# qianduoduolr/FGVC

Measured on AMD Instinct MI355X. Metric: frames/sec + ms/corr-volume, 480p 8-frame clip, 1/2/4/8 MI355X, higher is better.
Workload: dtype f16 + fp6 (e2m3) MFMA operands, f32 accumulate; top-k near-ties re-scored in f64 from f32 features

## Files before the change

### fgvc_amd/csrc/common.hpp

```cpp
#pragma once

#include <hip/hip_runtime.h>
#include <math.h>
#include <stdint.h>
#include <stdio.h>

#include "../../include/fgvc_hip.h"
#include "sortnet.hpp"

namespace fgvc {

typedef float f32x4 __attribute__((ext_vector_type(4)));
typedef float f32x16 __attribute__((ext_vector_type(16)));
typedef short bf16x8 __attribute__((ext_vector_type(8)));

constexpr int WAVE = 64;
constexpr int IDX_EMPTY = 0x7fffffff;

void set_error(const char* fmt, ...);

#define FGVC_REQUIRE(cond, code, ...)        \
  do {                                       \
    if (!(cond)) {                           \
      ::fgvc::set_error(__VA_ARGS__);        \
// ... 193 lines not shown
typedef int fgvc_i32x8 __attribute__((ext_vector_type(8)));
typedef int fgvc_i32x4 __attribute__((ext_vector_type(4)));

constexpr int F8_AX = 7, F8_BX = 3;
constexpr int F8_AW = 2, F8_BW = 9;

__device__ __forceinline__ void split_f16_4(const f32x4& x, float s, uint2& hw, uint32_t& l8, uint32_t& h8, uint2& lw, bool& ovf) {
  typedef _Float16 f16x4 __attribute__((ext_vector_type(4)));
  f16x4 h, l;
  float hf[4], lf[4];
#pragma unroll
  for (int i = 0; i < 4; ++i) {
    const float xs = x[i] * s;
    ovf |= fabsf(xs) > 57344.f;
    const float c = __builtin_amdgcn_fmed3f(xs, -65504.f, 65504.f);
    h[i] = (_Float16)c;
    hf[i] = (float)h[i];
    lf[i] = c - hf[i];
    l[i] = (_Float16)lf[i];
  }
  hw = __builtin_bit_cast(uint2, h);
  lw = __builtin_bit_cast(uint2, l);
  constexpr float SA = 1.0f / (float)(1 << F8_AX), SB = (float)(1 << F8_BX);
  int a = __builtin_amdgcn_cvt_pk_fp8_f32(__builtin_amdgcn_fmed3f(hf[0] * SA, -448.f, 448.f), __builtin_amdgcn_fmed3f(hf[1] * SA, -448.f, 448.f), 0, false);
  a = __builtin_amdgcn_cvt_pk_fp8_f32(__builtin_amdgcn_fmed3f(hf[2] * SA, -448.f, 448.f), __builtin_amdgcn_fmed3f(hf[3] * SA, -448.f, 448.f), a, true);
  int b = __builtin_amdgcn_cvt_pk_fp8_f32(lf[0] * SB, lf[1] * SB, 0, false);
  b = __builtin_amdgcn_cvt_pk_fp8_f32(lf[2] * SB, lf[3] * SB, b, true);
  h8 = (uint32_t)a;
  l8 = (uint32_t)b;
}

typedef int fgvc_i32x6 __attribute__((ext_vector_type(6)));
typedef int fgvc_i32x16 __attribute__((ext_vector_type(16)));
__device__ __forceinline__ void split_f16f6_chunk(const f32x4 (&v)[4], float s, int h, uint2 (&hw)[4], fgvc_i32x4& main6, fgvc_i32x4& tail6,
                                                  bool& ovf, float lo = -65504.f) {
  typedef _Float16 f16x2 __attribute__((ext_vector_type(2)));
  unsigned A[8], B[8];
  float mc = 0.f, md = 0.f;
#pragma unroll
  for (int g = 0; g < 4; ++g)
#pragma unroll
    for (int j = 0; j < 2; ++j) {
      const float c0 = __builtin_amdgcn_fmed3f(v[g][2 * j] * s, lo, 65504.f);
      const float c1 = __builtin_amdgcn_fmed3f(v[g][2 * j + 1] * s, lo, 65504.f);
      mc = fmaxf(fmaxf(mc, fabsf(c0)), fabsf(c1));
      f16x2 hp, lp;
      hp[0] = (_Float16)c0;
      hp[1] = (_Float16)c1;
      const float d0 = c0 - (float)hp[0], d1 = c1 - (float)hp[1];
      md = fmaxf(fmaxf(md, fabsf(d0)), fabsf(d1));
      lp[0] = (_Float16)(d0 * 2048.f);
      lp[1] = (_Float16)(d1 * 2048.f);
      A[2 * g + j] = __builtin_bit_cast(unsigned, hp);
      B[2 * g + j] = __builtin_bit_cast(unsigned, lp);
    }
  ovf |= mc > 57344.f;
  const float mh = (float)(_Float16)mc;
  const float ml = md * 2048.f;
#pragma unroll
  for (int g = 0; g < 4; ++g) hw[g] = {A[2 * g], A[2 * g + 1]};
#pragma unroll
  for (int r = 0; r < 8; ++r) {
    const auto t = __builtin_amdgcn_permlane32_swap(A[r], B[r], false, false);
    A[r] = t[0]; B[r] = t[1];
  }
  const auto tm = __builtin_amdgcn_permlane32_swap(__builtin_bit_cast(unsigned, mh), __builtin_bit_cast(unsigned, ml), false, false);
  const unsigned mu = tm[0] > tm[1] ? tm[0] : tm[1];
  const float m16 = (float)(_Float16)__builtin_bit_cast(float, mu);
  const unsigned mb = __builtin_bit_cast(unsigned, m16);
  int field = (int)(mb >> 23) - 2 + ((mb & 0x7fffffu) > 0x700000u ? 1 : 0);
  field = field < 32 ? 32 : field;
  fgvc_i32x16 T;
#pragma unroll
  for (int g = 0; g < 4; ++g)
#pragma unroll
    for (int j = 0; j < 2; ++j) {
      T[4 * g + j] = (int)A[2 * g + j];
      T[4 * g + 2 + j] = (int)B[2 * g + j];
    }
  fgvc_i32x6 c6;
  const unsigned sc_bits = (unsigned)field << 23;
  asm volatile("v_cvt_scalef32_pk32_fp6_f16 %0, %1, %2" : "=&v"(c6) : "v"(T), "v"(sc_bits));
  main6 = {c6[0], c6[1], c6[2], c6[3]};
  tail6 = {c6[4], c6[5], field - (h ? 11 : 0), 0};
}

__device__ __forceinline__ void lds_barrier() { asm volatile("s_waitcnt lgkmcnt(0)\n\ts_barrier" ::: "memory"); }

__host__ __device__ __forceinline__ int imin(int a, int b) { return a < b ? a : b; }
__host__ __device__ __forceinline__ int imax(int a, int b) { return a > b ? a : b; }
__host__ __device__ __forceinline__ int cdiv(int a, int b) { return (a + b - 1) / b; }

}
```

### fgvc_amd/csrc/conv_split.hip

```cpp
#include "common.hpp"

namespace fgvc {

struct ConvSplitParams {
  const uint16_t* x;
  const uint16_t* w;
  const float* bias;
  const float* residual;
  uint16_t* y_split;
  float* y_f32;
  int N, H, W, Hp, Wp, Cin, Cout, relu;
  int n_ty, n_tx;
  int debug;
  float acc_scale;
  float out_scale;
  int out_fmt;
  int* overflow;
  const uint16_t* x2;
  const uint16_t* w2;
  int Cin2;
  unsigned char* y_bank;
  int bank_normalize;
  int bank_row_bytes;
};
// ... 830 lines not shown
  for (int i = 0; i < 4; ++i) {
    ph |= n6_code(hf[i] * ih) << (6 * i);
    pl |= n6_code(lf[i] * il) << (6 * i);
  }
  const int v = lane >> 4, hi = (lane >> 1) & 1, pi = ((lane >> 2) & 3) * 2 + (lane & 1);
  const int w = pi < 6 ? pi : 0;
  const int pa = (4 * w) / 3, oa = 32 * w - 24 * pa;
  const int base = (lane & ~13) ;
  const int la = base + 4 * (pa >> 1) + (pa & 1), lb = base + 4 * ((pa + 1) >> 1) + ((pa + 1) & 1);
  const unsigned ha = __shfl(ph, la), hb = __shfl(ph, lb), qa = __shfl(pl, la), qb = __shfl(pl, lb);
  const unsigned wh = (ha >> oa) | (hb << (24 - oa)), wl = (qa >> oa) | (qb << (24 - oa));
  if (pi < 4) {
    *reinterpret_cast<unsigned*>(row + 512 + 32 * v + 16 * hi + 4 * pi) = wh;
    *reinterpret_cast<unsigned*>(row + 704 + 32 * v + 16 * hi + 4 * pi) = wl;
  } else if (pi < 6) {
    *reinterpret_cast<unsigned*>(row + 640 + 32 * (v >> 1) + 16 * hi + 8 * (v & 1) + 4 * (pi - 4)) = wh;
    *reinterpret_cast<unsigned*>(row + 832 + 32 * (v >> 1) + 16 * hi + 8 * (v & 1) + 4 * (pi - 4)) = wl;
  } else if (pi == 6) {
    row[896 + 16 * hi + v] = (unsigned char)(sh + 127 - 4);
  } else {
    row[896 + 16 * hi + 4 + v] = (unsigned char)(sl + 127 - 4);
  }
  if (lane < 2) *reinterpret_cast<unsigned long long*>(row + 904 + 16 * lane) = 0ull;
  else if (lane < 26) *reinterpret_cast<unsigned*>(row + 928 + 4 * (lane - 2)) = 0u;
}

static int g_conv_debug = 0;
void set_conv_debug(int v) { g_conv_debug = v; }
static int g_conv_narrow = 1;
void set_conv_narrow(int v) { g_conv_narrow = v; }
static int g_conv_cot_cap = 0;
void set_conv_cot_cap(int v) { g_conv_cot_cap = v; }

template <int COT, int OUT_FMT, bool RES, bool F32OUT, bool GENERIC, bool BANK = false, int CIN_TAG = 0>
__global__ __launch_bounds__(256, 1) void conv256p_kernel(ConvSplitParams p) {
  constexpr int NA = COT / 64, PPW = NA * 2;
  constexpr int TROWS = 8, PATCHB = (TROWS + 2) * CV_PW * 128, SLOTB = COT * 128, NPIECE = (TROWS + 2) * 5;
  __shared__ __attribute__((aligned(16))) unsigned char smem[PATCHB + 3 * SLOTB + COT * 4];
  unsigned char* patch = smem;
  unsigned char* wring = smem + PATCHB;
  float* bias_lds = reinterpret_cast<float*>(smem + PATCHB + 3 * SLOTB);
  const long long t_begin = __builtin_amdgcn_s_memtime();
  const int tid = threadIdx.x, lane = tid & 63;
  const int wave = __builtin_amdgcn_readfirstlane(tid >> 6);
  const int ch = wave & 1, pr = wave >> 1;
  const int n = lane & 31, h = lane >> 5;
  const int d_row = lane >> 3, d_slot = lane & 7;
  int bid = blockIdx.x;
  const int nimg = bid / (p.n_ty * p.n_tx);
  bid -= nimg * p.n_ty * p.n_tx;
  const int ty = bid / p.n_tx, tx = bid - ty * p.n_tx;
  const int y0 = ty * TROWS, x0 = tx * 32;
  const int co_base = blockIdx.y * COT;
  const int nchunk = p.Cin / 32;
  const uint32_t pixb = (uint32_t)nchunk * 128u;

  const uint32_t w_lane_off = (uint32_t)(d_row * 128 + ((d_slot ^ (d_row >> 1)) << 4));
  const uint32_t wo[2] = {w_lane_off, w_lane_off ^ 64u};
  const uint32_t ring_lds = lds_addr(wring), patch_lds = lds_addr(patch);
  const uint32_t wl = ring_lds + (uint32_t)((ch * (COT / 2) + n) * 128) + ((((uint32_t)h) ^ (uint32_t)((n >> 1) & 7)) << 4);
  uint32_t pl[3][2];
#pragma unroll
  for (int dx = 0; dx < 3; ++dx)
#pragma unroll
    for (int par = 0; par < 2; ++par) {
      const uint32_t key = (uint32_t)((((n + dx) >> 1) & 7) ^ (4 * par));
      pl[dx][par] = patch_lds + (uint32_t)((4 * pr * CV_PW + n + dx) * 128) + ((((uint32_t)h) ^ key) << 4);
    }
  const uint32_t pf_lane_off = (uint32_t)d_row * pixb + (uint32_t)((d_slot ^ (d_row >> 1)) << 4);
  const uint32_t lane16 = (uint32_t)lane * 16u;
  int ptab;
  {
    const int k = lane & 15, i = imin(wave + 4 * k, NPIECE - 1);
    const int prow = i / 5, pc0 = (i - prow * 5) * 8;
    const int goff = (int)((uint32_t)(prow * p.Wp + pc0) * pixb);
    const int ldst = (prow * CV_PW + pc0) * 128;
    const int key = ((prow + (pc0 >> 3)) & 1) << 6;
    ptab = lane < 16 ? goff : lane < 32 ? ldst : key;
  }
  const unsigned char* xb_tile = reinterpret_cast<const unsigned char*>(p.x) + (uint32_t)((nimg * p.Hp + y0) * p.Wp + x0) * pixb;
  const unsigned char* wb_tile = reinterpret_cast<const unsigned char*>(p.w) + (uint32_t)(co_base * 128);
  const uint32_t piece_off = (uint32_t)(wave * PPW * 1024);
  auto weight_base = [&](int chunk, int tap) { return wb_tile + (uint32_t)((tap * nchunk + chunk) * p.Cout * 128); };
  auto weight_piece = [&](const unsigned char* base, uint32_t dst, int j) {
    const unsigned char* src = base + piece_off + (uint32_t)(j * 1024);
    const uint32_t d = dst + piece_off + (uint32_t)(j * 1024);
    asm volatile("s_mov_b32 m0, %2\n\ts_nop 0\n\tglobal_load_lds_dwordx4 %0, %1" ::"v"(wo[j & 1]), "s"(src), "s"(d) : "memory");
  };

  if (tid < COT / 4) reinterpret_cast<f32x4*>(bias_lds)[tid] = reinterpret_cast<const f32x4*>(p.bias + co_base)[tid];
  for (int i = wave; i < NPIECE; i += 4) {
    const int prow = i / 5, pc0 = (i - prow * 5) * 8;
    const int P = prow * CV_PW + pc0 + d_row;
    const int sl = d_slot ^ ((P >> 1) & 7);
    const size_t gpix = ((size_t)nimg * p.Hp + (y0 + prow)) * p.Wp + (x0 + pc0 + d_row);
    conv_lds_dma_16(reinterpret_cast<const unsigned char*>(p.x) + gpix * pixb + sl * 16, lds_addr(patch + (prow * CV_PW + pc0) * 128));
  }
#pragma unroll
  for (int j = 0; j < PPW; ++j) weight_piece(weight_base(0, 0), ring_lds, j);
#pragma unroll
  for (int j = 0; j < PPW; ++j) weight_piece(weight_base(0, 1), ring_lds + SLOTB, j);

  __builtin_amdgcn_s_waitcnt(0x0F70);

  const long long t_loop0 = __builtin_amdgcn_s_memtime();
  {
    const size_t wb64 = (size_t)wb_tile, xb64 = (size_t)xb_tile;
    const int s_tap = __builtin_amdgcn_readfirstlane(nchunk * p.Cout * 128), s_chunk = __builtin_amdgcn_readfirstlane(p.Cout * 128);
    const int s_nchunk = __builtin_amdgcn_readfirstlane(nchunk), s_ring = __builtin_amdgcn_readfirstlane((int)ring_lds);
    const int s_patch = __builtin_amdgcn_readfirstlane((int)patch_lds), s_piece = __builtin_amdgcn_readfirstlane((int)piece_off);
    typedef int i32x2 __attribute__((ext_vector_type(2)));
    const i32x2 s_wb = {__builtin_amdgcn_readfirstlane((int)(uint32_t)wb64), __builtin_amdgcn_readfirstlane((int)(uint32_t)(wb64 >> 32))};
    const i32x2 s_xb = {__builtin_amdgcn_readfirstlane((int)(uint32_t)xb64), __builtin_amdgcn_readfirstlane((int)(uint32_t)(xb64 >> 32))};
    typedef int i32x2_t __attribute__((ext_vector_type(2)));
    i32x2_t loop_cycles;
    const int nchunk2 = p.x2 ? p.Cin2 / 32 : 0;
    const uint32_t pixb2 = (uint32_t)nchunk2 * 128u;
    const uint32_t pf_lane_off2 = (uint32_t)d_row * pixb2 + (uint32_t)((d_slot ^ (d_row >> 1)) << 4);
    int ptab2;
    {
      const int k2 = lane & 15, i2 = imin(wave + 4 * k2, NPIECE - 1);
      const int prow = i2 / 5, pc0 = (i2 - prow * 5) * 8;
      const int goff = (int)((uint32_t)(prow * p.Wp + pc0) * pixb2);
// ... 5 lines not shown
    const int s_last2 = __builtin_amdgcn_readfirstlane(nchunk2 ? nchunk - 1 : -1), s_nchunk2 = __builtin_amdgcn_readfirstlane(nchunk2);
#define C256P_INPUTS                                                                                                              \
  "{v232}"(wl), "{v233}"(pl[0][0]), "{v234}"(pl[0][1]), "{v235}"(pl[1][0]), "{v236}"(pl[1][1]), "{v237}"(pl[2][0]), "{v238}"(pl[2][1]),     \
      "{v239}"(wo[0]), "{v240}"(wo[1]), "{v241}"(pf_lane_off), "{v242}"(lane16), "{v243}"(ptab), "{v244}"(pf_lane_off2), "{v245}"(ptab2),  \
      "{s[20:21]}"(s_wb), "{s22}"(s_tap), "{s23}"(s_chunk), "{s[24:25]}"(s_xb), "{s26}"(s_nchunk), "{s27}"(s_ring), "{s28}"(s_patch),      \
      "{s29}"(s_piece), "{s46}"(s_last2), "{s[48:49]}"(s_w2b), "{s[50:51]}"(s_x2b), "{s52}"(s_nchunk2)
    if constexpr (COT == 256) {
#include "conv256p_loop.inc"
    } else {
#include "conv128p_loop.inc"
    }
#undef C256P_INPUTS
    if ((p.debug & 8) && blockIdx.x == 300 && blockIdx.y == 0 && lane == 0 && p.y_split) {
      long long* o = reinterpret_cast<long long*>(p.y_split) + wave * 8;
      o[4] = (long long)(uint32_t)loop_cycles.x | ((long long)loop_cycles.y << 32);
      o[5] = nchunk * 9 + nchunk2;
      o[0] = t_loop0 - t_begin;
    }
  }
  f32x16 acc[NA][4];
  if constexpr (NA == 4)
    asm volatile(""
                 : "={a[0:15]}"(acc[0][0]), "={a[16:31]}"(acc[0][1]), "={a[32:47]}"(acc[0][2]), "={a[48:63]}"(acc[0][3]), "={a[64:79]}"(acc[1][0]),
                   "={a[80:95]}"(acc[1][1]), "={a[96:111]}"(acc[1][2]), "={a[112:127]}"(acc[1][3]), "={a[128:143]}"(acc[NA - 2][0]),
                   "={a[144:159]}"(acc[NA - 2][1]), "={a[160:175]}"(acc[NA - 2][2]), "={a[176:191]}"(acc[NA - 2][3]), "={a[192:207]}"(acc[NA - 1][0]),
                   "={a[208:223]}"(acc[NA - 1][1]), "={a[224:239]}"(acc[NA - 1][2]), "={a[240:255]}"(acc[NA - 1][3]));
  else
    asm volatile(""
                 : "={a[0:15]}"(acc[0][0]), "={a[16:31]}"(acc[0][1]), "={a[32:47]}"(acc[0][2]), "={a[48:63]}"(acc[0][3]), "={a[64:79]}"(acc[1][0]),
                   "={a[80:95]}"(acc[1][1]), "={a[96:111]}"(acc[1][2]), "={a[112:127]}"(acc[1][3]));

  int lane_e;
  asm volatile("v_mbcnt_lo_u32_b32 %0, -1, 0\n\tv_mbcnt_hi_u32_b32 %0, -1, %0" : "=v"(lane_e));
  {
  int lane = lane_e, n = lane & 31, h = lane >> 5;
  int Wp_e = __builtin_amdgcn_readfirstlane(p.Wp);
  asm volatile("" : "+s"(Wp_e));
  constexpr int RPW = 4, CW = COT / 2, RB = CW * 4, RS = RB + 16, LPR = RB / 16, RPI = 64 / LPR;
  static_assert(4 * 32 * RS <= PATCHB + 3 * SLOTB, "epilogue staging");
  __syncthreads();
  long long ts0 = __builtin_amdgcn_s_memtime(), ts1 = 0, ts2 = 0, ts3 = 0, ts4 = 0;
  unsigned char* tile = smem + wave * (32 * RS);
  const int co_w = co_base + ch * CW;
  int mv_row = lane / LPR, mv_col = (lane % LPR) * 16;
  auto row_fence = [&]() { asm volatile("" : "+v"(n), "+v"(h), "+v"(mv_row), "+v"(mv_col)); };
  auto wave_sync = [&]() { asm volatile("s_waitcnt lgkmcnt(0)" ::: "memory"); };
  constexpr int RSLOTS = RB / 16, RPIECES = 32 * RB / 1024, RPPP = 1024 / RB;
  static_assert(4 * 32 * RS + 4 * 32 * RB <= PATCHB + 3 * SLOTB, "residual tiles");
  unsigned char* rtile = smem + 4 * (32 * RS) + wave * (32 * RB);
  const bool has_res = GENERIC || BANK ? p.residual != nullptr : RES;
  auto residual_dma = [&](int b_) {
    const int y_ = y0 + RPW * pr + b_;
    if (!has_res || b_ >= RPW || y_ >= p.H) return;
    const unsigned char* src = reinterpret_cast<const unsigned char*>(p.residual + (((size_t)nimg * p.H + y_) * p.W + x0) * p.Cout + co_w);
    const int pmax = p.W - 1 - x0;
#pragma unroll
    for (int j = 0; j < RPIECES; ++j) {
      const int pp = j * RPPP + (lane * 16) / RB, ps = ((lane * 16) % RB) / 16;
      const uint32_t voff = (uint32_t)(imin(pp, pmax) * p.Cout * 4 + ((ps ^ (pp & (RSLOTS - 1))) << 4));
      conv_lds_dma_16s(voff, src, lds_addr(rtile + j * 1024));
    }
  };
  auto residual_wait = [&](int stores_behind) {
    if (x0 + 32 > p.W || stores_behind == 0) asm volatile("s_waitcnt vmcnt(0)" ::: "memory");
    else if (stores_behind == 32 / RPI) asm volatile("s_waitcnt vmcnt(%0)" ::"n"(32 / RPI) : "memory");
    else asm volatile("s_waitcnt vmcnt(%0)" ::"n"(2 * (32 / RPI)) : "memory");
  };
  auto residual_at = [&](int cw) {
    return *reinterpret_cast<const f32x4*>(rtile + n * RB + ((((cw * 4) >> 4) ^ (n & (RSLOTS - 1))) << 4));
  };
  residual_dma(0);
  const bool tile_full = x0 + 32 <= p.W;
  auto store_rows = [&](unsigned char* dst) {
    unsigned char* d0 = dst + (size_t)mv_row * p.Cout * 4 + mv_col;
    const unsigned char* t0 = tile + mv_row * RS + mv_col;
    if (tile_full) {
#pragma unroll
      for (int i = 0; i < 32 / RPI; ++i) *reinterpret_cast<uint4*>(d0 + (size_t)(i * RPI) * p.Cout * 4) = *reinterpret_cast<const uint4*>(t0 + i * RPI * RS);
    } else {
#pragma unroll
      for (int i = 0; i < 32 / RPI; ++i)
        if (x0 + i * RPI + mv_row < p.W) *reinterpret_cast<uint4*>(d0 + (size_t)(i * RPI) * p.Cout * 4) = *reinterpret_cast<const uint4*>(t0 + i * RPI * RS);
    }
  };
  if constexpr (BANK) {
    {
      constexpr int BK_RS = 1024 + 16;
      static_assert(COT == 256 && 2 * 32 * BK_RS <= PATCHB + 3 * SLOTB, "bank staging");
      unsigned char* rows = smem + pr * (32 * BK_RS);
      float* part = reinterpret_cast<float*>(rows);
      long long bts[6] = {}, bt_begin = 0;
#pragma unroll
      for (int b = 0; b < RPW; ++b) {
        row_fence();
        const int y = y0 + RPW * pr + b;
        const bool row_ok = y < p.H;
        if (b == 1) bt_begin = __builtin_amdgcn_s_memtime();
        if (b == 2) bts[4] = __builtin_amdgcn_s_memtime();
        const size_t fpix0 = ((size_t)nimg * p.H + imin(y, p.H - 1)) * p.W + x0;
        if (has_res && row_ok) residual_wait(b == 0 || 32 / RPI != 16 ? 0 : (p.bank_row_bytes > 1024 ? 32 : 16));
        f32x4 v[NA][4];
#pragma unroll
        for (int a = 0; a < NA; ++a)
#pragma unroll
          for (int g = 0; g < 4; ++g) {
            const int cw = a * 32 + 8 * g + 4 * h;
            const f32x4 bv = *reinterpret_cast<const f32x4*>(bias_lds + ch * CW + cw);
            v[a][g] = {fmaf(acc[a][b][4 * g + 0], p.acc_scale, bv.x), fmaf(acc[a][b][4 * g + 1], p.acc_scale, bv.y),
                         fmaf(acc[a][b][4 * g + 2], p.acc_scale, bv.z), fmaf(acc[a][b][4 * g + 3], p.acc_scale, bv.w)};
            if (has_res && row_ok) v[a][g] += residual_at(cw);
            if (p.relu) {
              v[a][g].x = fmaxf(v[a][g].x, 0.f); v[a][g].y = fmaxf(v[a][g].y, 0.f);
              v[a][g].z = fmaxf(v[a][g].z, 0.f); v[a][g].w = fmaxf(v[a][g].w, 0.f);
            }
          }
        if (has_res) { wave_sync(); residual_dma(b + 1); }
        if (b == 1) bts[0] = __builtin_amdgcn_s_memtime();
        __syncthreads();
        float pp[NA][4];
        {
#pragma clang fp contract(off)
#pragma unroll
          for (int a = 0; a < NA; ++a)
#pragma unroll
            for (int g = 0; g < 4; ++g) {
              const float xx = v[a][g].x * v[a][g].x, yy = v[a][g].y * v[a][g].y, zz = v[a][g].z * v[a][g].z, ww = v[a][g].w * v[a][g].w;
              pp[a][g] = ((xx + yy) + zz) + ww;
              part[(ch * 16 + a * 4 + g) * 64 + lane] = pp[a][g];
            }
        }
        __syncthreads();
        float ss;
        {
          float t[NA][4];
#pragma unroll
          for (int a = 0; a < NA; ++a)
#pragma unroll
            for (int g = 0; g < 4; ++g) t[a][g] = pp[a][g] + part[((ch ^ 1) * 16 + a * 4 + g) * 64 + lane];
          float u[2][4], w4[4];
#pragma unroll
          for (int g = 0; g < 4; ++g) { u[0][g] = t[0][g] + t[2][g]; u[1][g] = t[1][g] + t[3][g]; }
#pragma unroll
          for (int g = 0; g < 4; ++g) w4[g] = u[0][g] + u[1][g];
          const float z0 = w4[0] + w4[2], z1 = w4[1] + w4[3];
          const float s1 = z0 + z1;
          ss = s1 + __shfl_xor(s1, 32);
        }
        __syncthreads();
        if (b == 1) bts[1] = __builtin_amdgcn_s_memtime();
        const float inv = p.bank_normalize ? 1.0f / fmaxf(sqrtf(ss), 1e-12f) : 1.0f;
        unsigned char* row = rows + n * BK_RS;
#pragma unroll
        for (int vl = 0; vl < 2; ++vl)
#pragma unroll
          for (int hi = 0; hi < 2; ++hi) {
            unsigned A_[16], B_[16];
            float mh = 0.f, ml = 0.f;
#pragma unroll
            for (int m = 0; m < 4; ++m) {
              const int a = 2 * vl + (m >> 1), g = hi + 2 * (m & 1);
              f32x4 x = v[a][g];
              x *= inv;
              typedef _Float16 f16x4 __attribute__((ext_vector_type(4)));
              f16x4 hv;
#pragma unroll
              for (int k = 0; k < 4; ++k) {
                const float xs = x[k] * 256.f;
                const _Float16 hh_ = (_Float16)xs;
                hv[k] = hh_;
                const float fh = (float)hh_, fl = (xs - fh) * 256.f;
                mh = fmaxf(mh, fabsf(fh)); ml = fmaxf(ml, fabsf(fl));
                A_[4 * m + k] = __builtin_bit_cast(unsigned, fh);
                B_[4 * m + k] = __builtin_bit_cast(unsigned, fl);
              }
              *reinterpret_cast<f16x4*>(row + 2 * (128 * ch + 32 * a + 8 * g + 4 * h)) = hv;
            }
#pragma unroll
            for (int j = 0; j < 16; ++j) {
              const auto t2 = __builtin_amdgcn_permlane32_swap(A_[j], B_[j], false, false);
              A_[j] = t2[0]; B_[j] = t2[1];
            }
            const auto tm = __builtin_amdgcn_permlane32_swap(__builtin_bit_cast(unsigned, mh), __builtin_bit_cast(unsigned, ml), false, false);
            const unsigned mb = tm[0] > tm[1] ? tm[0] : tm[1];
            int sexp = (int)(mb >> 23) - 129 + ((mb & 0x7fffffu) > 0x700000u ? 1 : 0);
            sexp = (mb == 0u || sexp < -40) ? -40 : sexp;
            fgvc_i32x16 S0, S1;
#pragma unroll
            for (int m = 0; m < 4; ++m) {
              S0[4 * m + 0] = (int)A_[4 * m + 0]; S0[4 * m + 1] = (int)A_[4 * m + 2]; S0[4 * m + 2] = (int)B_[4 * m + 0]; S0[4 * m + 3] = (int)B_[4 * m + 2];
              S1[4 * m + 0] = (int)A_[4 * m + 1]; S1[4 * m + 1] = (int)A_[4 * m + 3]; S1[4 * m + 2] = (int)B_[4 * m + 1]; S1[4 * m + 3] = (int)B_[4 * m + 3];
            }
            fgvc_i32x6 c6;
            const unsigned sc_bits = (unsigned)(sexp + 127) << 23;
            asm volatile("v_cvt_scalef32_2xpk16_fp6_f32 %0, %1, %2, %3" : "=&v"(c6) : "v"(S0), "v"(S1), "v"(sc_bits));
            const int vg = 2 * ch + vl;
            *reinterpret_cast<i32x4*>(row + (h ? 704 : 512) + 32 * vg + 16 * hi) = i32x4{c6[0], c6[1], c6[2], c6[3]};
            *reinterpret_cast<uint2*>(row + (h ? 832 : 640) + 32 * (vg >> 1) + 16 * hi + 8 * (vg & 1)) = uint2{(unsigned)c6[4], (unsigned)c6[5]};
            row[896 + 16 * hi + 4 * h + vg] = (unsigned char)(sexp + 127 - 4);
          }
        if (ch == 0) {
          if (h == 0) {
            *reinterpret_cast<unsigned long long*>(row + 904) = 0ull;
            *reinterpret_cast<unsigned long long*>(row + 920) = 0ull;
          } else {
#pragma unroll
            for (int i = 0; i < 6; ++i) *reinterpret_cast<i32x4*>(row + 928 + 16 * i) = i32x4{0, 0, 0, 0};
          }
        }
        if (b == 1) bts[2] = __builtin_amdgcn_s_memtime();
        __syncthreads();
        if (row_ok) {
          unsigned char* dst = p.y_bank + fpix0 * p.bank_row_bytes;
          if (x0 + 32 <= p.W) {
#pragma unroll
            for (int i = 0; i < 16; ++i) {
              const int r = 16 * ch + i;
              *reinterpret_cast<uint4*>(dst + (size_t)r * p.bank_row_bytes + 16 * lane) = *reinterpret_cast<const uint4*>(rows + r * BK_RS + 16 * lane);
            }
          } else {
#pragma unroll
            for (int i = 0; i < 16; ++i) {
              const int r = 16 * ch + i;
              if (x0 + r < p.W)
                *reinterpret_cast<uint4*>(dst + (size_t)r * p.bank_row_bytes + 16 * lane) = *reinterpret_cast<const uint4*>(rows + r * BK_RS + 16 * lane);
            }
          }
        }
        __syncthreads();
        if (b == 1) bts[3] = __builtin_amdgcn_s_memtime();
        if (p.bank_row_bytes > 1024) {
#pragma unroll
          for (int a = 0; a < NA; ++a)
#pragma unroll
            for (int g = 0; g < 4; ++g) {
              f32x4 x = v[a][g];
              x *= inv;
              *reinterpret_cast<f32x4*>(row + 4 * (128 * ch + 32 * a + 8 * g + 4 * h)) = x;
            }
          __syncthreads();
          if (row_ok) {
            unsigned char* dst = p.y_bank + fpix0 * p.bank_row_bytes + 1024;
            if (x0 + 32 <= p.W) {
#pragma unroll
              for (int i = 0; i < 16; ++i) {
                const int r = 16 * ch + i;
                *reinterpret_cast<uint4*>(dst + (size_t)r * p.bank_row_bytes + 16 * lane) = *reinterpret_cast<const uint4*>(rows + r * BK_RS + 16 * lane);
              }
            } else {
#pragma unroll
              for (int i = 0; i < 16; ++i) {
                const int r = 16 * ch + i;
                if (x0 + r < p.W)
                  *reinterpret_cast<uint4*>(dst + (size_t)r * p.bank_row_bytes + 16 * lane) = *reinterpret_cast<const uint4*>(rows + r * BK_RS + 16 * lane);
              }
            }
          }
          __syncthreads();
        }
      }
      if ((p.debug & 8) && blockIdx.x == 300 && blockIdx.y == 0 && lane == 0) {
        long long* o_ = reinterpret_cast<long long*>(p.y_bank) + wave * 8;
        o_[0] = bts[0] - bt_begin; o_[1] = bts[1] - bts[0]; o_[2] = bts[2] - bts[1]; o_[3] = bts[3] - bts[2]; o_[4] = bts[4] - bts[3]; o_[5] = __builtin_amdgcn_s_memtime() - t_begin;
      }
      return;
    }
  }
  constexpr bool HOIST_BIAS = false;
  constexpr bool FUSE_RELU = !GENERIC && !F32OUT && OUT_FMT == 3;
  const float clamp_lo = __builtin_bit_cast(float, __builtin_amdgcn_readfirstlane(FUSE_RELU && p.relu ? 0 : (int)0xC77FE000u));
  f32x4 bvv[HOIST_BIAS ? NA : 1][4];
  if constexpr (HOIST_BIAS) {
#pragma unroll
    for (int a = 0; a < NA; ++a)
#pragma unroll
      for (int g = 0; g < 4; ++g) bvv[a][g] = *reinterpret_cast<const f32x4*>(bias_lds + ch * CW + a * 32 + 8 * g + 4 * h);
  }
#pragma unroll
  for (int b = 0; b < RPW; ++b) {
    row_fence();
    const int y = y0 + RPW * pr + b;
    if (y >= p.H) continue;
    const size_t pix0 = ((size_t)nimg * p.Hp + (y + 1)) * Wp_e + (x0 + 1);
    const size_t fpix0 = ((size_t)nimg * p.H + y) * p.W + x0;
    if (has_res) residual_wait(b == 0 ? 0 : ((GENERIC ? p.y_f32 != nullptr : F32OUT) ? 32 / RPI : 0) + (p.y_split ? 32 / RPI : 0));
    f32x4 v[NA][4];
#pragma unroll
    for (int a = 0; a < NA; ++a)
#pragma unroll
      for (int g = 0; g < 4; ++g) {
        const int cw = a * 32 + 8 * g + 4 * h;
        const f32x4 bv = HOIST_BIAS ? bvv[HOIST_BIAS ? a : 0][g] : *reinterpret_cast<const f32x4*>(bias_lds + ch * CW + cw);
        v[a][g] = {fmaf(acc[a][b][4 * g + 0], p.acc_scale, bv.x), fmaf(acc[a][b][4 * g + 1], p.acc_scale, bv.y),
                   fmaf(acc[a][b][4 * g + 2], p.acc_scale, bv.z), fmaf(acc[a][b][4 * g + 3], p.acc_scale, bv.w)};
        if (has_res) v[a][g] += residual_at(cw);
        if (p.relu && !FUSE_RELU) {
          v[a][g].x = fmaxf(v[a][g].x, 0.f); v[a][g].y = fmaxf(v[a][g].y, 0.f);
          v[a][g].z = fmaxf(v[a][g].z, 0.f); v[a][g].w = fmaxf(v[a][g].w, 0.f);
        }
      }
    if (has_res) { wave_sync(); residual_dma(b + 1); }
    if (b == 1) { asm volatile("s_nop 0" ::"v"(v[0][0]), "v"(v[3][3])); ts1 = __builtin_amdgcn_s_memtime(); }
    if (GENERIC ? p.y_f32 != nullptr : F32OUT) {
      wave_sync();
#pragma unroll
      for (int a = 0; a < NA; ++a)
#pragma unroll
        for (int g = 0; g < 4; ++g) *reinterpret_cast<f32x4*>(tile + n * RS + (a * 32 + 8 * g + 4 * h) * 4) = v[a][g];
      wave_sync();
      store_rows(reinterpret_cast<unsigned char*>(p.y_f32 + fpix0 * p.Cout + co_w));
    }
    if (p.y_split) {
      wave_sync();
      const int out_fmt = GENERIC ? p.out_fmt : OUT_FMT;
      if (out_fmt == 0) {
#pragma unroll
        for (int a = 0; a < NA; ++a)
#pragma unroll
          for (int g = 0; g < 4; ++g) {
            ushort4 hv, lv;
            split_bf16_4(v[a][g], hv, lv);
            unsigned char* o = tile + n * RS + a * 128 + (8 * g + 4 * h) * 2;
            *reinterpret_cast<ushort4*>(o) = hv;
            *reinterpret_cast<ushort4*>(o + 64) = lv;
          }
      } else if (out_fmt == 3) {
        bool ovf = false;
#pragma unroll
        for (int a = 0; a < NA; ++a) {
          uint2 hw[4];
          i32x4 main6, tail6;
          split_f16f6_chunk(v[a], p.out_scale, h, hw, main6, tail6, ovf, clamp_lo);
          unsigned char* o = tile + n * RS + a * 128;
#pragma unroll
          for (int g = 0; g < 4; ++g) *reinterpret_cast<uint2*>(o + (8 * g + 4 * h) * 2) = hw[g];
          *reinterpret_cast<i32x4*>(o + 80 - 16 * h) = main6;
          *reinterpret_cast<i32x4*>(o + 112 - 16 * h) = tail6;
        }
        if (__builtin_amdgcn_ballot_w64(ovf && x0 + n < p.W) != 0ull && lane == 0) atomicOr(p.overflow, 1);
      } else {
        bool ovf = false;
#pragma unroll
        for (int a = 0; a < NA; ++a)
#pragma unroll
          for (int g = 0; g < 4; ++g) {
            uint2 hw, lw;
            uint32_t l8, h8;
            split_f16_4(v[a][g], p.out_scale, hw, l8, h8, lw, ovf);
            unsigned char* o = tile + n * RS + a * 128;
            *reinterpret_cast<uint2*>(o + (8 * g + 4 * h) * 2) = hw;
            if (out_fmt == 1) {
              *reinterpret_cast<uint32_t*>(o + 64 + 8 * g + 4 * h) = l8;
              *reinterpret_cast<uint32_t*>(o + 96 + 8 * g + 4 * h) = h8;
            } else {
              *reinterpret_cast<uint2*>(o + 64 + (8 * g + 4 * h) * 2) = lw;
            }
          }
        if (__builtin_amdgcn_ballot_w64(ovf && x0 + n < p.W) != 0ull && lane == 0) atomicOr(p.overflow, 1);
      }
      wave_sync();
      if (b == 1) ts2 = __builtin_amdgcn_s_memtime();
      store_rows(reinterpret_cast<unsigned char*>(p.y_split) + (pix0 * (p.Cout / 32) + (co_w >> 5)) * 128);
    }
    wave_sync();
    if (b == 0) ts4 = __builtin_amdgcn_s_memtime();
    if (b == 1) ts3 = __builtin_amdgcn_s_memtime();
  }
  if ((p.debug & 8) && blockIdx.x == 300 && blockIdx.y == 0 && lane == 0 && p.y_split) {
    long long* o_ = reinterpret_cast<long long*>(p.y_split) + wave * 8;
    o_[2] = ts4 - ts0; o_[3] = ts1 - ts4; o_[6] = ts2 - ts1; o_[7] = ts3 - ts2;
    asm volatile("s_waitcnt vmcnt(0)" ::: "memory");
    reinterpret_cast<long long*>(p.y_split)[wave * 8 + 1] = __builtin_amdgcn_s_memtime() - t_begin;
  }
  }
}

template <int ARITH>
static void conv_split_dispatch(const ConvSplitParams& p, dim3 grid, int KS, int cot_eff, bool narrow, hipStream_t s) {
  if (KS == 3) {
    if (cot_eff == 256 && p.y_bank) conv_split_kernel<3, 256, 1, 3, 4, false, ARITH, 2, true><<<grid, 512, 0, s>>>(p);
    else if (cot_eff == 256 && p.x2) conv_split_kernel<3, 256, 1, 3, 4, false, ARITH, 2, false, true><<<grid, 512, 0, s>>>(p);
    else if (cot_eff == 256) conv_split_kernel<3, 256, 1, 3, 4, false, ARITH><<<grid, 512, 0, s>>>(p);
    else if (cot_eff == 128 && narrow) conv_split_kernel<3, 128, 1, 3, 2, false, ARITH><<<grid, 256, 0, s>>>(p);
    else if (cot_eff == 128) conv_split_kernel<3, 128, 3, 2, 4, false, ARITH><<<grid, 512, 0, s>>>(p);
    else if (narrow) conv_split_kernel<3, 64, 3, 2, 2, false, ARITH><<<grid, 256, 0, s>>>(p);
    else conv_split_kernel<3, 64, 3, 3, 4, false, ARITH><<<grid, 512, 0, s>>>(p);
  } else {
    if (cot_eff == 256) conv_split_kernel<1, 256, 1, 3, 4, false, ARITH><<<grid, 512, 0, s>>>(p);
    else if (cot_eff == 128) conv_split_kernel<1, 128, 1, 3, 4, false, ARITH><<<grid, 512, 0, s>>>(p);
    else if (narrow) conv_split_kernel<1, 64, 1, 3, 2, false, ARITH><<<grid, 256, 0, s>>>(p);
    else conv_split_kernel<1, 64, 1, 3, 4, false, ARITH><<<grid, 512, 0, s>>>(p);
  }
}

int conv_split_launch(const uint16_t* x, const uint16_t* w, const float* bias, const float* residual, uint16_t* y_split,
                      float* y_f32, int N, int H, int W, int Hp, int Wp, int Cin, int Cout, int KS, int relu, int in_fmt,
                      int in_scale_log2, int out_fmt, int out_scale_log2, int* overflow, hipStream_t s, unsigned char* y_bank,
                      int bank_normalize, const uint16_t* x2, const uint16_t* w2, int Cin2, int bank_row_bytes) {
  ConvSplitParams p;
  p.x = x; p.w = w; p.bias = bias; p.residual = residual; p.y_split = y_split; p.y_f32 = y_f32;
  p.N = N; p.H = H; p.W = W; p.Hp = Hp; p.Wp = Wp; p.Cin = Cin; p.Cout = Cout; p.relu = relu;
  p.acc_scale = ldexpf(1.0f, -in_scale_log2); p.out_scale = ldexpf(1.0f, out_scale_log2); p.out_fmt = out_fmt; p.overflow = overflow;
  p.y_bank = y_bank; p.bank_normalize = bank_normalize; p.bank_row_bytes = bank_row_bytes;
  p.x2 = x2; p.w2 = w2; p.Cin2 = Cin2;
  const int cot = (Cout % 256 == 0) ? 256 : (Cout % 128 == 0) ? 128 : 64;
  const int cot_eff = (g_conv_cot_cap && cot > g_conv_cot_cap && !y_bank && !x2) ? g_conv_cot_cap : cot;
  const bool narrow = (cot_eff == 64 && (g_conv_narrow & 1)) || (cot_eff == 128 && KS == 3 && (g_conv_narrow & 2));
  p.n_ty = cdiv(H, narrow ? 4 : 8); p.n_tx = cdiv(W, 32);
  p.debug = g_conv_debug;
  dim3 grid(p.n_ty * p.n_tx * N, Cout / cot_eff);
  const bool fits32 = (unsigned long long)N * Hp * Wp * (Cin / 32) * 128ull < (1ull << 32) && (unsigned long long)9 * Cin * Cout * 4ull < (1ull << 32) &&
                      (!x2 || ((unsigned long long)N * Hp * Wp * (Cin2 / 32) * 128ull < (1ull << 32) && (unsigned long long)Cin2 * Cout * 4ull < (1ull << 32)));
  if (in_fmt == 3 && KS == 3 && (cot_eff == 256 || cot_eff == 128) && !narrow && (!y_bank || (cot_eff == 256 && !x2)) && (!x2 || (cot_eff == 256 && Cin2 >= 32)) &&
      Cin >= 32 && fits32 && !(g_conv_debug & 1024)) {
    if (y_bank) conv256p_kernel<256, -1, false, false, true, true><<<grid, 256, 0, s>>>(p);
    else if (cot_eff == 256) {
      if (y_split && out_fmt == 3 && !residual && !y_f32 && p.Cin == 128) conv256p_kernel<256, 3, false, false, false, false, 1><<<grid, 256, 0, s>>>(p);
      else if (y_split && out_fmt == 3 && !residual && !y_f32) conv256p_kernel<256, 3, false, false, false><<<grid, 256, 0, s>>>(p);
      else if (y_split && out_fmt == 3 && !residual && y_f32) conv256p_kernel<256, 3, false, true, false><<<grid, 256, 0, s>>>(p);
      else if (y_split && out_fmt == 3 && residual && y_f32) conv256p_kernel<256, 3, true, true, false><<<grid, 256, 0, s>>>(p);
      else if (y_split && out_fmt == 3 && residual && !y_f32) conv256p_kernel<256, 3, true, false, false><<<grid, 256, 0, s>>>(p);
      else conv256p_kernel<256, -1, false, false, true><<<grid, 256, 0, s>>>(p);
    } else {
      if (y_split && out_fmt == 3 && !residual && !y_f32) conv256p_kernel<128, 3, false, false, false><<<grid, 256, 0, s>>>(p);
      else if (y_split && out_fmt == 3 && residual && y_f32) conv256p_kernel<128, 3, true, true, false><<<grid, 256, 0, s>>>(p);
      else if (y_split && out_fmt == 3 && residual && !y_f32) conv256p_kernel<128, 3, true, false, false><<<grid, 256, 0, s>>>(p);
      else conv256p_kernel<128, -1, false, false, true><<<grid, 256, 0, s>>>(p);
    }
    FGVC_CHECK_LAUNCH("fgvc_conv_split_f32");
    return FGVC_OK;
  }
  if (in_fmt == 1) conv_split_dispatch<1>(p, grid, KS, cot_eff, narrow, s);
  else if (in_fmt == 3) conv_split_dispatch<3>(p, grid, KS, cot_eff, narrow, s);
  else if (in_fmt == 2) conv_split_dispatch<2>(p, grid, KS, cot_eff, narrow, s);
  else if (KS == 3 && cot_eff == 256 && !(g_conv_debug & 16) && !y_bank && !x2) conv_split_kernel<3, 256, 1, 3, 4, true><<<grid, 512, 0, s>>>(p);
  else conv_split_dispatch<0>(p, grid, KS, cot_eff, narrow, s);
  FGVC_CHECK_LAUNCH("fgvc_conv_split_f32");
  return FGVC_OK;
}

int nchw_to_split_nhwc_launch(const float* in, uint16_t* out, float* out_f32, int N, int C, int H, int W, int Hp, int Wp,
                              hipStream_t s) {
  dim3 grid(cdiv(W, 256), H, N * (C / 32));
  nchw_to_split_nhwc_kernel<<<grid, 256, 0, s>>>(in, out, out_f32, C, H, W, Hp, Wp);
  FGVC_CHECK_LAUNCH("fgvc_nchw_to_split_nhwc_f32");
  return FGVC_OK;
}

// ... 42 lines not shown
```

Baseline: 1998.

## Fold output scale into bias and accumulator scale; batch bias reads in conv epilogue

In the conv256p epilogue the output scale is folded into the bias (scaled when staged to LDS) and into the accumulator scale, so the f16/fp6 split no longer multiplies by the scale. Bias is now read with one batched block of ds_read_b128 per row instead of per-group loads. Accumulators are read through explicit accvgpr reads, and v_fma_mix is used for the f16 residual. A specialised bank-epilogue instantiation (BANKT) hard-wires residual, relu, normalize and 2048-byte rows so those runtime branches drop out. These changes trade more register pressure (v255 clobber, 16 live bias vectors) and inline asm for fewer VALU and LDS operations per output row, and folding the scale may change rounding slightly.

Result: no change. 2002 (median of 6 runs) (+0.2%).

```diff
diff --git a/fgvc_amd/csrc/common.hpp b/fgvc_amd/csrc/common.hpp
--- a/fgvc_amd/csrc/common.hpp
+++ b/fgvc_amd/csrc/common.hpp
@@ -249,8 +249,8 @@
 
 typedef int fgvc_i32x6 __attribute__((ext_vector_type(6)));
 typedef int fgvc_i32x16 __attribute__((ext_vector_type(16)));
-__device__ __forceinline__ void split_f16f6_chunk(const f32x4 (&v)[4], float s, int h, uint2 (&hw)[4], fgvc_i32x4& main6, fgvc_i32x4& tail6,
-                                                  bool& ovf, float lo = -65504.f) {
+__device__ __forceinline__ void split_f16f6_scaled(const f32x4 (&cs)[4], int h, uint2 (&hw)[4], fgvc_i32x4& main6, fgvc_i32x4& tail6, bool& ovf,
+                                                   float lo = -65504.f) {
   typedef _Float16 f16x2 __attribute__((ext_vector_type(2)));
   unsigned A[8], B[8];
   float mc = 0.f, md = 0.f;
@@ -258,17 +258,23 @@
   for (int g = 0; g < 4; ++g)
 #pragma unroll
     for (int j = 0; j < 2; ++j) {
-      const float c0 = __builtin_amdgcn_fmed3f(v[g][2 * j] * s, lo, 65504.f);
-      const float c1 = __builtin_amdgcn_fmed3f(v[g][2 * j + 1] * s, lo, 65504.f);
+      const float c0 = __builtin_amdgcn_fmed3f(cs[g][2 * j], lo, 65504.f);
+      const float c1 = __builtin_amdgcn_fmed3f(cs[g][2 * j + 1], lo, 65504.f);
       mc = fmaxf(fmaxf(mc, fabsf(c0)), fabsf(c1));
       f16x2 hp, lp;
       hp[0] = (_Float16)c0;
       hp[1] = (_Float16)c1;
-      const float d0 = c0 - (float)hp[0], d1 = c1 - (float)hp[1];
+      const unsigned hpu = __builtin_bit_cast(unsigned, hp);
+      fgvc_f32x2 d;
+      float d0, d1;
+      asm("v_fma_mix_f32 %0, -%1, 1.0, %2 op_sel_hi:[1,0,0]" : "=v"(d0) : "v"(hpu), "v"(c0));
+      asm("v_fma_mix_f32 %0, -%1, 1.0, %2 op_sel:[1,0,0] op_sel_hi:[1,0,0]" : "=v"(d1) : "v"(hpu), "v"(c1));
+      d = {d0, d1};
       md = fmaxf(fmaxf(md, fabsf(d0)), fabsf(d1));
-      lp[0] = (_Float16)(d0 * 2048.f);
-      lp[1] = (_Float16)(d1 * 2048.f);
-      A[2 * g + j] = __builtin_bit_cast(unsigned, hp);
+      d *= 2048.f;
+      lp[0] = (_Float16)d[0];
+      lp[1] = (_Float16)d[1];
+      A[2 * g + j] = hpu;
       B[2 * g + j] = __builtin_bit_cast(unsigned, lp);
     }
   ovf |= mc > 57344.f;
@@ -301,6 +307,13 @@
   main6 = {c6[0], c6[1], c6[2], c6[3]};
   tail6 = {c6[4], c6[5], field - (h ? 11 : 0), 0};
 }
+__device__ __forceinline__ void split_f16f6_chunk(const f32x4 (&v)[4], float s, int h, uint2 (&hw)[4], fgvc_i32x4& main6, fgvc_i32x4& tail6,
+                                                  bool& ovf, float lo = -65504.f) {
+  f32x4 cs[4];
+#pragma unroll
+  for (int g = 0; g < 4; ++g) cs[g] = v[g] * s;
+  split_f16f6_scaled(cs, h, hw, main6, tail6, ovf, lo);
+}
 
 __device__ __forceinline__ void lds_barrier() { asm volatile("s_waitcnt lgkmcnt(0)\n\ts_barrier" ::: "memory"); }
 
diff --git a/fgvc_amd/csrc/conv_split.hip b/fgvc_amd/csrc/conv_split.hip
--- a/fgvc_amd/csrc/conv_split.hip
+++ b/fgvc_amd/csrc/conv_split.hip
@@ -886,7 +886,7 @@
 static int g_conv_cot_cap = 0;
 void set_conv_cot_cap(int v) { g_conv_cot_cap = v; }
 
-template <int COT, int OUT_FMT, bool RES, bool F32OUT, bool GENERIC, bool BANK = false, int CIN_TAG = 0>
+template <int COT, int OUT_FMT, bool RES, bool F32OUT, bool GENERIC, bool BANK = false, int CIN_TAG = 0, bool BANKT = false>
 __global__ __launch_bounds__(256, 1) void conv256p_kernel(ConvSplitParams p) {
   constexpr int NA = COT / 64, PPW = NA * 2;
   constexpr int TROWS = 8, PATCHB = (TROWS + 2) * CV_PW * 128, SLOTB = COT * 128, NPIECE = (TROWS + 2) * 5;
@@ -942,7 +942,12 @@
     asm volatile("s_mov_b32 m0, %2\n\ts_nop 0\n\tglobal_load_lds_dwordx4 %0, %1" ::"v"(wo[j & 1]), "s"(src), "s"(d) : "memory");
   };
 
-  if (tid < COT / 4) reinterpret_cast<f32x4*>(bias_lds)[tid] = reinterpret_cast<const f32x4*>(p.bias + co_base)[tid];
+  constexpr bool FUSE_RELU = !GENERIC && !F32OUT && OUT_FMT == 3;
+  if (tid < COT / 4) {
+    f32x4 bq = reinterpret_cast<const f32x4*>(p.bias + co_base)[tid];
+    if constexpr (FUSE_RELU) bq *= p.out_scale;
+    reinterpret_cast<f32x4*>(bias_lds)[tid] = bq;
+  }
   for (int i = wave; i < NPIECE; i += 4) {
     const int prow = i / 5, pc0 = (i - prow * 5) * 8;
     const int P = prow * CV_PW + pc0 + d_row;
@@ -1014,6 +1019,7 @@
 
   int lane_e;
   asm volatile("v_mbcnt_lo_u32_b32 %0, -1, 0\n\tv_mbcnt_hi_u32_b32 %0, -1, %0" : "=v"(lane_e));
+  if constexpr (COT == 256) asm volatile("" ::: "v255");
   {
   int lane = lane_e, n = lane & 31, h = lane >> 5;
   int Wp_e = __builtin_amdgcn_readfirstlane(p.Wp);
@@ -1030,7 +1036,8 @@
   constexpr int RSLOTS = RB / 16, RPIECES = 32 * RB / 1024, RPPP = 1024 / RB;
   static_assert(4 * 32 * RS + 4 * 32 * RB <= PATCHB + 3 * SLOTB, "residual tiles");
   unsigned char* rtile = smem + 4 * (32 * RS) + wave * (32 * RB);
-  const bool has_res = GENERIC || BANK ? p.residual != nullptr : RES;
+  static_assert(!BANKT || BANK, "BANKT names a form of the bank epilogue");
+  const bool has_res = BANKT ? true : GENERIC || BANK ? p.residual != nullptr : RES;
   auto residual_dma = [&](int b_) {
     const int y_ = y0 + RPW * pr + b_;
     if (!has_res || b_ >= RPW || y_ >= p.H) return;
@@ -1065,6 +1072,35 @@
         if (x0 + i * RPI + mv_row < p.W) *reinterpret_cast<uint4*>(d0 + (size_t)(i * RPI) * p.Cout * 4) = *reinterpret_cast<const uint4*>(t0 + i * RPI * RS);
     }
   };
+#define C256P_ACC4(T, G)                                                                                                                 \
+  ({                                                                                                                                     \
+    float x_, y_, z_, w_;                                                                                                                \
+    asm volatile("v_accvgpr_read_b32 %0, %4\n\tv_accvgpr_read_b32 %1, %5\n\tv_accvgpr_read_b32 %2, %6\n\tv_accvgpr_read_b32 %3, %7"      \
+                 : "=v"(x_), "=v"(y_), "=v"(z_), "=v"(w_)                                                                                \
+                 : "a"((T)[4 * (G)]), "a"((T)[4 * (G) + 1]), "a"((T)[4 * (G) + 2]), "a"((T)[4 * (G) + 3]));                              \
+    f32x4{x_, y_, z_, w_};                                                                                                               \
+  })
+  auto bias_row = [&](f32x4 (&bv)[NA][4]) {
+    const uint32_t ba = lds_addr(bias_lds + ch * CW + 4 * h);
+    if constexpr (NA == 4)
+      asm volatile("ds_read_b128 %0, %16\n\tds_read_b128 %1, %16 offset:32\n\tds_read_b128 %2, %16 offset:64\n\tds_read_b128 %3, %16 offset:96\n\t"
+                   "ds_read_b128 %4, %16 offset:128\n\tds_read_b128 %5, %16 offset:160\n\tds_read_b128 %6, %16 offset:192\n\tds_read_b128 %7, %16 offset:224\n\t"
+                   "ds_read_b128 %8, %16 offset:256\n\tds_read_b128 %9, %16 offset:288\n\tds_read_b128 %10, %16 offset:320\n\tds_read_b128 %11, %16 offset:352\n\t"
+                   "ds_read_b128 %12, %16 offset:384\n\tds_read_b128 %13, %16 offset:416\n\tds_read_b128 %14, %16 offset:448\n\tds_read_b128 %15, %16 offset:480\n\t"
+                   "s_waitcnt lgkmcnt(0)"
+                   : "=&v"(bv[0][0]), "=&v"(bv[0][1]), "=&v"(bv[0][2]), "=&v"(bv[0][3]), "=&v"(bv[1][0]), "=&v"(bv[1][1]), "=&v"(bv[1][2]), "=&v"(bv[1][3]),
+                     "=&v"(bv[NA - 2][0]), "=&v"(bv[NA - 2][1]), "=&v"(bv[NA - 2][2]), "=&v"(bv[NA - 2][3]), "=&v"(bv[NA - 1][0]), "=&v"(bv[NA - 1][1]),
+                     "=&v"(bv[NA - 1][2]), "=&v"(bv[NA - 1][3])
+                   : "v"(ba)
+                   : "memory");
+    else
+      asm volatile("ds_read_b128 %0, %8\n\tds_read_b128 %1, %8 offset:32\n\tds_read_b128 %2, %8 offset:64\n\tds_read_b128 %3, %8 offset:96\n\t"
+                   "ds_read_b128 %4, %8 offset:128\n\tds_read_b128 %5, %8 offset:160\n\tds_read_b128 %6, %8 offset:192\n\tds_read_b128 %7, %8 offset:224\n\t"
+                   "s_waitcnt lgkmcnt(0)"
+                   : "=&v"(bv[0][0]), "=&v"(bv[0][1]), "=&v"(bv[0][2]), "=&v"(bv[0][3]), "=&v"(bv[1][0]), "=&v"(bv[1][1]), "=&v"(bv[1][2]), "=&v"(bv[1][3])
+                   : "v"(ba)
+                   : "memory");
+  };
   if constexpr (BANK) {
     {
       constexpr int BK_RS = 1024 + 16;
@@ -1072,6 +1108,8 @@
       unsigned char* rows = smem + pr * (32 * BK_RS);
       float* part = reinterpret_cast<float*>(rows);
       long long bts[6] = {}, bt_begin = 0;
+      const bool bk_relu = BANKT || p.relu, bk_norm = BANKT || p.bank_normalize;
+      const int bk_row_bytes = BANKT ? 2048 : p.bank_row_bytes;
 #pragma unroll
       for (int b = 0; b < RPW; ++b) {
         row_fence();
@@ -1080,18 +1118,19 @@
         if (b == 1) bt_begin = __builtin_amdgcn_s_memtime();
         if (b == 2) bts[4] = __builtin_amdgcn_s_memtime();
         const size_t fpix0 = ((size_t)nimg * p.H + imin(y, p.H - 1)) * p.W + x0;
-        if (has_res && row_ok) residual_wait(b == 0 || 32 / RPI != 16 ? 0 : (p.bank_row_bytes > 1024 ? 32 : 16));
+        if (has_res && row_ok) residual_wait(b == 0 || 32 / RPI != 16 ? 0 : (bk_row_bytes > 1024 ? 32 : 16));
+        f32x4 bvs[NA][4];
+        bias_row(bvs);
         f32x4 v[NA][4];
 #pragma unroll
         for (int a = 0; a < NA; ++a)
 #pragma unroll
           for (int g = 0; g < 4; ++g) {
             const int cw = a * 32 + 8 * g + 4 * h;
-            const f32x4 bv = *reinterpret_cast<const f32x4*>(bias_lds + ch * CW + cw);
-            v[a][g] = {fmaf(acc[a][b][4 * g + 0], p.acc_scale, bv.x), fmaf(acc[a][b][4 * g + 1], p.acc_scale, bv.y),
-                         fmaf(acc[a][b][4 * g + 2], p.acc_scale, bv.z), fmaf(acc[a][b][4 * g + 3], p.acc_scale, bv.w)};
+            const f32x4 bv = bvs[a][g], av = C256P_ACC4(acc[a][b], g);
+            v[a][g] = {fmaf(av.x, p.acc_scale, bv.x), fmaf(av.y, p.acc_scale, bv.y), fmaf(av.z, p.acc_scale, bv.z), fmaf(av.w, p.acc_scale, bv.w)};
             if (has_res && row_ok) v[a][g] += residual_at(cw);
-            if (p.relu) {
+            if (bk_relu) {
               v[a][g].x = fmaxf(v[a][g].x, 0.f); v[a][g].y = fmaxf(v[a][g].y, 0.f);
               v[a][g].z = fmaxf(v[a][g].z, 0.f); v[a][g].w = fmaxf(v[a][g].w, 0.f);
             }
@@ -1130,7 +1169,7 @@
         }
         __syncthreads();
         if (b == 1) bts[1] = __builtin_amdgcn_s_memtime();
-        const float inv = p.bank_normalize ? 1.0f / fmaxf(sqrtf(ss), 1e-12f) : 1.0f;
+        const float inv = bk_norm ? 1.0f / fmaxf(sqrtf(ss), 1e-12f) : 1.0f;
         unsigned char* row = rows + n * BK_RS;
 #pragma unroll
         for (int vl = 0; vl < 2; ++vl)
@@ -1192,25 +1231,25 @@
         if (b == 1) bts[2] = __builtin_amdgcn_s_memtime();
         __syncthreads();
         if (row_ok) {
-          unsigned char* dst = p.y_bank + fpix0 * p.bank_row_bytes;
+          unsigned char* dst = p.y_bank + fpix0 * bk_row_bytes;
           if (x0 + 32 <= p.W) {
 #pragma unroll
             for (int i = 0; i < 16; ++i) {
               const int r = 16 * ch + i;
-              *reinterpret_cast<uint4*>(dst + (size_t)r * p.bank_row_bytes + 16 * lane) = *reinterpret_cast<const uint4*>(rows + r * BK_RS + 16 * lane);
+              *reinterpret_cast<uint4*>(dst + (size_t)r * bk_row_bytes + 16 * lane) = *reinterpret_cast<const uint4*>(rows + r * BK_RS + 16 * lane);
             }
           } else {
 #pragma unroll
             for (int i = 0; i < 16; ++i) {
               const int r = 16 * ch + i;
               if (x0 + r < p.W)
-                *reinterpret_cast<uint4*>(dst + (size_t)r * p.bank_row_bytes + 16 * lane) = *reinterpret_cast<const uint4*>(rows + r * BK_RS + 16 * lane);
+                *reinterpret_cast<uint4*>(dst + (size_t)r * bk_row_bytes + 16 * lane) = *reinterpret_cast<const uint4*>(rows + r * BK_RS + 16 * lane);
             }
           }
         }
         __syncthreads();
         if (b == 1) bts[3] = __builtin_amdgcn_s_memtime();
-        if (p.bank_row_bytes > 1024) {
+        if (bk_row_bytes > 1024) {
 #pragma unroll
           for (int a = 0; a < NA; ++a)
 #pragma unroll
@@ -1221,19 +1260,19 @@
             }
           __syncthreads();
           if (row_ok) {
-            unsigned char* dst = p.y_bank + fpix0 * p.bank_row_bytes + 1024;
+            unsigned char* dst = p.y_bank + fpix0 * bk_row_bytes + 1024;
             if (x0 + 32 <= p.W) {
 #pragma unroll
               for (int i = 0; i < 16; ++i) {
                 const int r = 16 * ch + i;
-                *reinterpret_cast<uint4*>(dst + (size_t)r * p.bank_row_bytes + 16 * lane) = *reinterpret_cast<const uint4*>(rows + r * BK_RS + 16 * lane);
+                *reinterpret_cast<uint4*>(dst + (size_t)r * bk_row_bytes + 16 * lane) = *reinterpret_cast<const uint4*>(rows + r * BK_RS + 16 * lane);
               }
             } else {
 #pragma unroll
               for (int i = 0; i < 16; ++i) {
                 const int r = 16 * ch + i;
                 if (x0 + r < p.W)
-                  *reinterpret_cast<uint4*>(dst + (size_t)r * p.bank_row_bytes + 16 * lane) = *reinterpret_cast<const uint4*>(rows + r * BK_RS + 16 * lane);
+                  *reinterpret_cast<uint4*>(dst + (size_t)r * bk_row_bytes + 16 * lane) = *reinterpret_cast<const uint4*>(rows + r * BK_RS + 16 * lane);
               }
             }
           }
@@ -1247,16 +1286,8 @@
       return;
     }
   }
-  constexpr bool HOIST_BIAS = false;
-  constexpr bool FUSE_RELU = !GENERIC && !F32OUT && OUT_FMT == 3;
   const float clamp_lo = __builtin_bit_cast(float, __builtin_amdgcn_readfirstlane(FUSE_RELU && p.relu ? 0 : (int)0xC77FE000u));
-  f32x4 bvv[HOIST_BIAS ? NA : 1][4];
-  if constexpr (HOIST_BIAS) {
-#pragma unroll
-    for (int a = 0; a < NA; ++a)
-#pragma unroll
-      for (int g = 0; g < 4; ++g) bvv[a][g] = *reinterpret_cast<const f32x4*>(bias_lds + ch * CW + a * 32 + 8 * g + 4 * h);
-  }
+  const float acc_scale_e = FUSE_RELU ? p.acc_scale * p.out_scale : p.acc_scale;
 #pragma unroll
   for (int b = 0; b < RPW; ++b) {
     row_fence();
@@ -1265,16 +1296,20 @@
     const size_t pix0 = ((size_t)nimg * p.Hp + (y + 1)) * Wp_e + (x0 + 1);
     const size_t fpix0 = ((size_t)nimg * p.H + y) * p.W + x0;
     if (has_res) residual_wait(b == 0 ? 0 : ((GENERIC ? p.y_f32 != nullptr : F32OUT) ? 32 / RPI : 0) + (p.y_split ? 32 / RPI : 0));
+    f32x4 bvs[NA][4];
+    bias_row(bvs);
     f32x4 v[NA][4];
 #pragma unroll
     for (int a = 0; a < NA; ++a)
 #pragma unroll
       for (int g = 0; g < 4; ++g) {
         const int cw = a * 32 + 8 * g + 4 * h;
-        const f32x4 bv = HOIST_BIAS ? bvv[HOIST_BIAS ? a : 0][g] : *reinterpret_cast<const f32x4*>(bias_lds + ch * CW + cw);
-        v[a][g] = {fmaf(acc[a][b][4 * g + 0], p.acc_scale, bv.x), fmaf(acc[a][b][4 * g + 1], p.acc_scale, bv.y),
-                   fmaf(acc[a][b][4 * g + 2], p.acc_scale, bv.z), fmaf(acc[a][b][4 * g + 3], p.acc_scale, bv.w)};
-        if (has_res) v[a][g] += residual_at(cw);
+        const f32x4 bv = bvs[a][g], av = C256P_ACC4(acc[a][b], g);
+        v[a][g] = __builtin_elementwise_fma(av, f32x4{acc_scale_e, acc_scale_e, acc_scale_e, acc_scale_e}, bv);
+        if (has_res) {
+          if constexpr (FUSE_RELU) v[a][g] = __builtin_elementwise_fma(residual_at(cw), f32x4{p.out_scale, p.out_scale, p.out_scale, p.out_scale}, v[a][g]);
+          else v[a][g] += residual_at(cw);
+        }
         if (p.relu && !FUSE_RELU) {
           v[a][g].x = fmaxf(v[a][g].x, 0.f); v[a][g].y = fmaxf(v[a][g].y, 0.f);
           v[a][g].z = fmaxf(v[a][g].z, 0.f); v[a][g].w = fmaxf(v[a][g].w, 0.f);
@@ -1311,7 +1346,8 @@
         for (int a = 0; a < NA; ++a) {
           uint2 hw[4];
           i32x4 main6, tail6;
-          split_f16f6_chunk(v[a], p.out_scale, h, hw, main6, tail6, ovf, clamp_lo);
+          if constexpr (FUSE_RELU) split_f16f6_scaled(v[a], h, hw, main6, tail6, ovf, clamp_lo);
+          else split_f16f6_chunk(v[a], p.out_scale, h, hw, main6, tail6, ovf, clamp_lo);
           unsigned char* o = tile + n * RS + a * 128;
 #pragma unroll
           for (int g = 0; g < 4; ++g) *reinterpret_cast<uint2*>(o + (8 * g + 4 * h) * 2) = hw[g];
@@ -1353,6 +1389,7 @@
     asm volatile("s_waitcnt vmcnt(0)" ::: "memory");
     reinterpret_cast<long long*>(p.y_split)[wave * 8 + 1] = __builtin_amdgcn_s_memtime() - t_begin;
   }
+#undef C256P_ACC4
   }
 }
 
@@ -1394,7 +1431,8 @@
                       (!x2 || ((unsigned long long)N * Hp * Wp * (Cin2 / 32) * 128ull < (1ull << 32) && (unsigned long long)Cin2 * Cout * 4ull < (1ull << 32)));
   if (in_fmt == 3 && KS == 3 && (cot_eff == 256 || cot_eff == 128) && !narrow && (!y_bank || (cot_eff == 256 && !x2)) && (!x2 || (cot_eff == 256 && Cin2 >= 32)) &&
       Cin >= 32 && fits32 && !(g_conv_debug & 1024)) {
-    if (y_bank) conv256p_kernel<256, -1, false, false, true, true><<<grid, 256, 0, s>>>(p);
+    if (y_bank && residual && relu && bank_normalize && bank_row_bytes == 2048) conv256p_kernel<256, -1, false, false, true, true, 0, true><<<grid, 256, 0, s>>>(p);
+    else if (y_bank) conv256p_kernel<256, -1, false, false, true, true><<<grid, 256, 0, s>>>(p);
     else if (cot_eff == 256) {
       if (y_split && out_fmt == 3 && !residual && !y_f32 && p.Cin == 128) conv256p_kernel<256, 3, false, false, false, false, 1><<<grid, 256, 0, s>>>(p);
       else if (y_split && out_fmt == 3 && !residual && !y_f32) conv256p_kernel<256, 3, false, false, false><<<grid, 256, 0, s>>>(p);
```
